# jgrss/cultionet

Hardware: AMD Instinct MI355X
Metric: train_chips_per_sec (higher is better)
Workload: dtype f32

## Files before the change

### cultionet_amd/csrc/cn_norm.hip

```cpp
#include "cn_common.h"

#define BN_SPLIT_MAX 256
#define BN_SPLIT_GROUP 64

__global__ __launch_bounds__(256) void cn_bn_partial_kernel(const float* __restrict__ x, long xbs, int B, int C,
                                                           int L, int splits, double* __restrict__ part, int vec4) {
  __shared__ double scratch[4];
  const int c = blockIdx.x, sp = blockIdx.y;
  double s = 0.0, ss = 0.0;
  if (vec4) {
    const int L4 = L >> 2;
    const int per = (L4 + splits - 1) / splits;
    const int beg = sp * per;
    const int end = (beg + per < L4) ? beg + per : L4;
    for (int b = 0; b < B; ++b) {
      const float4* xp = reinterpret_cast<const float4*>(x + b * xbs + (long)c * L);
      for (int l = beg + threadIdx.x; l < end; l += 256) {
        const float4 v = xp[l];
        s += ((double)v.x + (double)v.y) + ((double)v.z + (double)v.w);
        ss += (double)v.x * v.x + (double)v.y * v.y + (double)v.z * v.z + (double)v.w * v.w;
      }
    }
  } else {
    const int per = (L + splits - 1) / splits;
// ... 21 lines not shown
  __shared__ double scratch[4];
  double a = 0.0, b = 0.0;
  for (int i = threadIdx.x; i < splits; i += 256) {
    a += part[((long)c * splits + i) * 2 + 0];
    b += part[((long)c * splits + i) * 2 + 1];
  }
  s = cn_block_sum<double, 256>(a, scratch);
  ss = cn_block_sum<double, 256>(b, scratch);
}

__global__ void cn_bn_eval_stats_kernel(const float* __restrict__ running_mean, const float* __restrict__ running_var,
                                        int C, float eps, float* __restrict__ mean, float* __restrict__ rstd) {
  const int c = blockIdx.x * blockDim.x + threadIdx.x;
  if (c >= C) return;
  mean[c] = running_mean[c];
  rstd[c] = 1.0f / sqrtf(running_var[c] + eps);
}

__global__ __launch_bounds__(256) void cn_bn_apply_kernel(const float* __restrict__ x, long xbs,
                                                         float* __restrict__ mean, float* __restrict__ rstd,
                                                         const float* __restrict__ gamma,
                                                         const float* __restrict__ beta,
                                                         const float* __restrict__ res, long rbs,
                                                         float* __restrict__ y, long ybs, int B, int C, int L, int act,
                                                         const double* __restrict__ part, int splits, double count,
                                                         float eps, float momentum, float* __restrict__ running_mean,
                                                         float* __restrict__ running_var) {
  const int c = blockIdx.y, b = blockIdx.z;
  float m, rs;
  if (part != nullptr) {
    double s, ss;
    cn_bn_sum_parts(part, c, splits, s, ss);
    const double md = s / count;
    double var = ss / count - md * md;
    if (var < 0.0) var = 0.0;
    m = (float)md;
    rs = (float)(1.0 / sqrt(var + (double)eps));
    if (blockIdx.x == 0 && b == 0 && threadIdx.x == 0) {
      mean[c] = m;
      rstd[c] = rs;
      if (running_mean != nullptr) {
        const double unbiased = count > 1.0 ? var * count / (count - 1.0) : var;
        running_mean[c] = (1.f - momentum) * running_mean[c] + momentum * m;
        running_var[c] = (1.f - momentum) * running_var[c] + momentum * (float)unbiased;
      }
    }
  } else {
    m = mean[c];
    rs = rstd[c];
  }
  const float sc = gamma[c] * rs, be = beta[c];
  const long r0 = (long)c * L;
  const float* xp = x + b * xbs + r0;
  const float* rp = res ? res + b * rbs + r0 : nullptr;
  float* yp = y + b * ybs + r0;
  for (int l = blockIdx.x * 256 + threadIdx.x; l < L; l += gridDim.x * 256) {
    float z = (xp[l] - m) * sc + be;
    if (act == 1) z = cn_silu(z);
    if (rp) z += rp[l];
    yp[l] = z;
  }
}

__global__ __launch_bounds__(256) void cn_bn_bwd_partial_kernel(const float* __restrict__ x, long xbs,
                                                               const float* __restrict__ dy, long dybs,
                                                               const float* __restrict__ mean,
                                                               const float* __restrict__ rstd,
                                                               const float* __restrict__ gamma,
                                                               const float* __restrict__ beta, int B, int C, int L,
                                                               int act, int splits, double* __restrict__ part,
                                                               int vec4) {
  __shared__ double scratch[4];
  const int c = blockIdx.x, sp = blockIdx.y;
  const float m = mean[c], rs = rstd[c], ga = gamma[c], be = beta[c];
  double s1 = 0.0, s2 = 0.0;
  auto term = [&](float xv, float dv) {
    const float xh = (xv - m) * rs;
    float dz = dv;
    if (act == 1) dz *= cn_silu_grad(ga * xh + be);
    s1 += dz;
    s2 += (double)dz * xh;
  };
  if (vec4) {
    const int L4 = L >> 2;
    const int per = (L4 + splits - 1) / splits;
    const int beg = sp * per;
    const int end = (beg + per < L4) ? beg + per : L4;
    for (int b = 0; b < B; ++b) {
      const float4* xp = reinterpret_cast<const float4*>(x + b * xbs + (long)c * L);
      const float4* dp = reinterpret_cast<const float4*>(dy + b * dybs + (long)c * L);
      for (int l = beg + threadIdx.x; l < end; l += 256) {
        const float4 xv = xp[l], dv = dp[l];
        term(xv.x, dv.x); term(xv.y, dv.y); term(xv.z, dv.z); term(xv.w, dv.w);
      }
    }
  } else {
    const int per = (L + splits - 1) / splits;
    const int beg = sp * per;
    const int end = (beg + per < L) ? beg + per : L;
    for (int b = 0; b < B; ++b) {
      const float* xp = x + b * xbs + (long)c * L;
      const float* dp = dy + b * dybs + (long)c * L;
      for (int l = beg + threadIdx.x; l < end; l += 256) term(xp[l], dp[l]);
    }
  }
  s1 = cn_block_sum<double, 256>(s1, scratch);
  s2 = cn_block_sum<double, 256>(s2, scratch);
  if (threadIdx.x == 0) {
    part[((long)c * splits + sp) * 2 + 0] = s1;
    part[((long)c * splits + sp) * 2 + 1] = s2;
  }
}

__global__ __launch_bounds__(256) void cn_bn_bwd_apply_kernel(const float* __restrict__ x, long xbs,
                                                             const float* __restrict__ dy, long dybs,
                                                             const float* __restrict__ mean,
                                                             const float* __restrict__ rstd,
                                                             const float* __restrict__ gamma,
                                                             const float* __restrict__ beta,
                                                             const double* __restrict__ part, int splits,
                                                             double count, int training,
                                                             float* __restrict__ dgamma, float* __restrict__ dbeta,
                                                             int accumulate_params, float* __restrict__ dx, long dxbs,
                                                             int B, int C, int L, int act, int accumulate) {
  const int c = blockIdx.y, b = blockIdx.z;
  double s1, s2;
  cn_bn_sum_parts(part, c, splits, s1, s2);
  if (blockIdx.x == 0 && b == 0 && threadIdx.x == 0) {
    if (accumulate_params) {
      dgamma[c] += (float)s2;
      dbeta[c] += (float)s1;
    } else {
      dgamma[c] = (float)s2;
      dbeta[c] = (float)s1;
    }
  }
  if (dx == nullptr) return;
  const float m = mean[c], rs = rstd[c], ga = gamma[c], be = beta[c];
  const float c1 = training ? (float)(s1 / count) : 0.f, c2 = training ? (float)(s2 / count) : 0.f;
  const long r0 = (long)c * L;
  const float* xp = x + b * xbs + r0;
  const float* dp = dy + b * dybs + r0;
  float* dxp = dx + b * dxbs + r0;
  for (int l = blockIdx.x * 256 + threadIdx.x; l < L; l += gridDim.x * 256) {
    const float xh = (xp[l] - m) * rs;
    float dz = dp[l];
    if (act == 1) dz *= cn_silu_grad(ga * xh + be);
    float g = (dz - c1 - xh * c2) * (ga * rs);
    if (accumulate) g += dxp[l];
    dxp[l] = g;
  }
}

template <int NV>
__global__ __launch_bounds__(256) void cn_bn_fused_fwd_kernel(const float* __restrict__ x, long xbs,
                                                             float* __restrict__ mean, float* __restrict__ rstd,
                                                             const float* __restrict__ gamma,
                                                             const float* __restrict__ beta,
                                                             const float* __restrict__ res, long rbs,
                                                             float* __restrict__ y, long ybs, int B, int C, int L,
                                                             int act, float eps, float momentum,
                                                             float* __restrict__ running_mean,
                                                             float* __restrict__ running_var) {
  __shared__ double scratch[4];
  const int c = blockIdx.x, n = B * L;
  float v[NV];
  double s = 0.0, ss = 0.0;
#pragma unroll
  for (int k = 0; k < NV; ++k) {
    const int i = threadIdx.x + k * 256;
    v[k] = 0.f;
    if (i < n) {
      const int b = i / L, l = i - b * L;
      v[k] = x[b * xbs + (long)c * L + l];
      s += v[k];
      ss += (double)v[k] * v[k];
    }
  }
  s = cn_block_sum<double, 256>(s, scratch);
  ss = cn_block_sum<double, 256>(ss, scratch);
  const double count = (double)n;
  const double md = s / count;
  double var = ss / count - md * md;
  if (var < 0.0) var = 0.0;
  const float m = (float)md, rs = (float)(1.0 / sqrt(var + (double)eps));
  if (threadIdx.x == 0) {
    mean[c] = m;
    rstd[c] = rs;
    if (running_mean != nullptr) {
      const double unbiased = count > 1.0 ? var * count / (count - 1.0) : var;
      running_mean[c] = (1.f - momentum) * running_mean[c] + momentum * m;
      running_var[c] = (1.f - momentum) * running_var[c] + momentum * (float)unbiased;
    }
  }
  const float sc = gamma[c] * rs, be = beta[c];
#pragma unroll
  for (int k = 0; k < NV; ++k) {
    const int i = threadIdx.x + k * 256;
    if (i < n) {
      const int b = i / L, l = i - b * L;
      float z = (v[k] - m) * sc + be;
      if (act == 1) z = cn_silu(z);
      if (res) z += res[b * rbs + (long)c * L + l];
      y[b * ybs + (long)c * L + l] = z;
    }
  }
}

template <int NV>
__global__ __launch_bounds__(256) void cn_bn_fused_bwd_kernel(const float* __restrict__ x, long xbs,
                                                             const float* __restrict__ dy, long dybs,
                                                             const float* __restrict__ mean,
                                                             const float* __restrict__ rstd,
                                                             const float* __restrict__ gamma,
                                                             const float* __restrict__ beta, int training,
                                                             float* __restrict__ dgamma, float* __restrict__ dbeta,
                                                             int accumulate_params, float* __restrict__ dx, long dxbs,
                                                             int B, int C, int L, int act, int accumulate) {
  __shared__ double scratch[4];
  const int c = blockIdx.x, n = B * L;
  const float m = mean[c], rs = rstd[c], ga = gamma[c], be = beta[c];
  float xh[NV], dz[NV];
  double s1 = 0.0, s2 = 0.0;
#pragma unroll
  for (int k = 0; k < NV; ++k) {
    const int i = threadIdx.x + k * 256;
    xh[k] = 0.f;
    dz[k] = 0.f;
    if (i < n) {
      const int b = i / L, l = i - b * L;
      xh[k] = (x[b * xbs + (long)c * L + l] - m) * rs;
      float d = dy[b * dybs + (long)c * L + l];
      if (act == 1) d *= cn_silu_grad(ga * xh[k] + be);
      dz[k] = d;
      s1 += d;
      s2 += (double)d * xh[k];
    }
  }
  s1 = cn_block_sum<double, 256>(s1, scratch);
  s2 = cn_block_sum<double, 256>(s2, scratch);
  if (threadIdx.x == 0) {
    if (accumulate_params) {
      dgamma[c] += (float)s2;
      dbeta[c] += (float)s1;
    } else {
      dgamma[c] = (float)s2;
      dbeta[c] = (float)s1;
    }
  }
  if (dx == nullptr) return;
  const double count = (double)n;
  const float c1 = training ? (float)(s1 / count) : 0.f, c2 = training ? (float)(s2 / count) : 0.f;
#pragma unroll
  for (int k = 0; k < NV; ++k) {
    const int i = threadIdx.x + k * 256;
    if (i < n) {
      const int b = i / L, l = i - b * L;
      float g = (dz[k] - c1 - xh[k] * c2) * (ga * rs);
      float* o = dx + b * dxbs + (long)c * L + l;
      if (accumulate) g += *o;
      *o = g;
    }
  }
}

#define BN_FUSED_MAX (8 * 256)

static int bn_splits_wide(int C, long L) {
  int s = (2048 + C - 1) / C;
  const long maxs = (L + 511) / 512;
  if (s > maxs) s = (int)maxs;
  if (s > BN_SPLIT_MAX) s = BN_SPLIT_MAX;
  if (s < 1) s = 1;
  return s;
}

static int bn_splits(int C, long L) {
  int s = (1024 + C - 1) / C;
  const long maxs = (L + 511) / 512;
  if (s > maxs) s = (int)maxs;
  if (s > BN_SPLIT_GROUP) s = BN_SPLIT_GROUP;
  if (s < 1) s = 1;
  return s;
}

static dim3 plane_grid(int B, int C, int L) {
  int bx = (L + 1023) / 1024;
  if (bx < 1) bx = 1;
  return dim3(bx, C, B);
}

extern "C" int cn_bn_workspace_doubles(int C) { return C * BN_SPLIT_MAX * 2; }

extern "C" int cn_bn_act_fwd_f32(const float* x, long xbs, const float* gamma, const float* beta,
                                 float* running_mean, float* running_var, const float* res, long rbs, float* y,
                                 long ybs, float* mean, float* rstd, double* ws, int B, int C, int L, int training,
                                 float momentum, float eps, int act, void* stream_) {
  hipStream_t stream = (hipStream_t)stream_;
  if (B <= 0 || C <= 0 || L <= 0) return CN_OK;
  if (training && (long)B * L <= BN_FUSED_MAX && C >= 32) {
#define CN_BN_FWD(NV_)                                                                                               \
  CN_LAUNCH((cn_bn_fused_fwd_kernel<NV_>), dim3(C), dim3(256), 0, stream, x, xbs, mean, rstd, gamma, beta, res, \
                     rbs, y, ybs, B, C, L, act, eps, momentum, running_mean, running_var)
    CN_BN_FWD(8);
#undef CN_BN_FWD
    return cn_check_launch();
  }
  if (training) {
    const int splits = bn_splits_wide(C, L);
    CN_LAUNCH(cn_bn_partial_kernel, dim3(C, splits), dim3(256), 0, stream, x, xbs, B, C, L, splits, ws,
                       (int)(L % 4 == 0 && xbs % 4 == 0 && (reinterpret_cast<uintptr_t>(x) & 15) == 0));
    CN_LAUNCH(cn_bn_apply_kernel, plane_grid(B, C, L), dim3(256), 0, stream, x, xbs, mean, rstd, gamma, beta,
                       res, rbs, y, ybs, B, C, L, act, (const double*)ws, splits, (double)B * L, eps, momentum,
                       running_mean, running_var);
  } else {
    CN_LAUNCH(cn_bn_eval_stats_kernel, dim3((C + 63) / 64), dim3(64), 0, stream, running_mean,
                       running_var, C, eps, mean, rstd);
    CN_LAUNCH(cn_bn_apply_kernel, plane_grid(B, C, L), dim3(256), 0, stream, x, xbs, mean, rstd, gamma, beta,
                       res, rbs, y, ybs, B, C, L, act, (const double*)nullptr, 0, 1.0, eps, momentum,
                       (float*)nullptr, (float*)nullptr);
  }
  return cn_check_launch();
}

extern "C" int cn_bn_act_bwd_f32(const float* x, long xbs, const float* dy, long dybs, const float* mean,
                                 const float* rstd, const float* gamma, const float* beta, float* dx, long dxbs,
                                 float* dgamma, float* dbeta, float* coef, double* ws, int B, int C, int L,
                                 int training, int act, int accumulate_dx, int accumulate_params, void* stream_) {
  hipStream_t stream = (hipStream_t)stream_;
  if (B <= 0 || C <= 0 || L <= 0) return CN_OK;
  if ((long)B * L <= BN_FUSED_MAX && C >= 32) {
#define CN_BN_BWD(NV_)                                                                                              \
  CN_LAUNCH((cn_bn_fused_bwd_kernel<NV_>), dim3(C), dim3(256), 0, stream, x, xbs, dy, dybs, mean, rstd, gamma, \
                     beta, training, dgamma, dbeta, accumulate_params, dx, dxbs, B, C, L, act, accumulate_dx)
    CN_BN_BWD(8);
#undef CN_BN_BWD
    return cn_check_launch();
  }
  const int splits = bn_splits_wide(C, L);
  CN_LAUNCH(cn_bn_bwd_partial_kernel, dim3(C, splits), dim3(256), 0, stream, x, xbs, dy, dybs, mean, rstd,
                     gamma, beta, B, C, L, act, splits, ws,
                     (int)(L % 4 == 0 && xbs % 4 == 0 && dybs % 4 == 0 &&
                           ((reinterpret_cast<uintptr_t>(x) | reinterpret_cast<uintptr_t>(dy)) & 15) == 0));
  (void)coef;
  CN_LAUNCH(cn_bn_bwd_apply_kernel, dx != nullptr ? plane_grid(B, C, L) : dim3(1, C, 1), dim3(256), 0,
                     stream, x, xbs, dy, dybs, mean, rstd, gamma, beta, (const double*)ws, splits, (double)B * L,
                     training, dgamma, dbeta, accumulate_params, dx, dxbs, B, C, L, act, accumulate_dx);
  return cn_check_launch();
}

#define BN_MAX_GROUPS 4
struct CnBnGroupArgs {
  const float* x[BN_MAX_GROUPS];
  const float* gamma[BN_MAX_GROUPS];
  const float* beta[BN_MAX_GROUPS];
  float* mean[BN_MAX_GROUPS];
  float* rstd[BN_MAX_GROUPS];
  float* running_mean[BN_MAX_GROUPS];
  float* running_var[BN_MAX_GROUPS];
  float* y[BN_MAX_GROUPS];
  const float* dy[BN_MAX_GROUPS];
  float* dx[BN_MAX_GROUPS];
  float* dgamma[BN_MAX_GROUPS];
  float* dbeta[BN_MAX_GROUPS];
  int accumulate_dx[BN_MAX_GROUPS];
  long xbs, ybs, dybs, dxbs, rbs;
  const float* res;
  int G, B, C, L, act, splits, training, sum_outputs, accumulate_params;
  int vec4;
  float eps, momentum;
  double* part;
};

__global__ __launch_bounds__(256) void cn_bn_group_partial_kernel(const CnBnGroupArgs a) {
  __shared__ double scratch[4];
  const int c = blockIdx.x, sp = blockIdx.y, g = blockIdx.z;
  double s = 0.0, ss = 0.0;
  if (a.vec4) {
    const int L4 = a.L >> 2;
    const int per = (L4 + a.splits - 1) / a.splits;
    const int beg = sp * per;
    const int end = (beg + per < L4) ? beg + per : L4;
    for (int b = 0; b < a.B; ++b) {
      const float4* xp = reinterpret_cast<const float4*>(a.x[g] + b * a.xbs + (long)c * a.L);
      for (int l = beg + threadIdx.x; l < end; l += 256) {
        const float4 v = xp[l];
        s += ((double)v.x + (double)v.y) + ((double)v.z + (double)v.w);
        ss += (double)v.x * v.x + (double)v.y * v.y + (double)v.z * v.z + (double)v.w * v.w;
      }
    }
  } else {
    const int per = (a.L + a.splits - 1) / a.splits;
    const int beg = sp * per;
    const int end = (beg + per < a.L) ? beg + per : a.L;
    for (int b = 0; b < a.B; ++b) {
      const float* xp = a.x[g] + b * a.xbs + (long)c * a.L;
      for (int l = beg + threadIdx.x; l < end; l += 256) {
        const float v = xp[l];
        s += v;
        ss += (double)v * v;
      }
    }
  }
  s = cn_block_sum<double, 256>(s, scratch);
  ss = cn_block_sum<double, 256>(ss, scratch);
  if (threadIdx.x == 0) {
    double* p = a.part + (((long)g * a.C + c) * a.splits + sp) * 2;
    p[0] = s;
    p[1] = ss;
  }
}

__global__ __launch_bounds__(256) void cn_bn_group_apply_kernel(const CnBnGroupArgs a) {
  const int c = blockIdx.y, b = blockIdx.z;
  float m[BN_MAX_GROUPS], sc[BN_MAX_GROUPS], be[BN_MAX_GROUPS];
  const double count = (double)a.B * a.L;
#pragma unroll
  for (int g = 0; g < BN_MAX_GROUPS; ++g) {
    m[g] = sc[g] = be[g] = 0.f;
    if (g < a.G) {
      float rs;
      if (a.training) {
        double s = 0.0, ss = 0.0;
        const double* p = a.part + ((long)g * a.C + c) * a.splits * 2;
        for (int i = 0; i < a.splits; ++i) {
          s += p[2 * i];
          ss += p[2 * i + 1];
        }
        const double md = s / count;
        double var = ss / count - md * md;
        if (var < 0.0) var = 0.0;
        m[g] = (float)md;
        rs = (float)(1.0 / sqrt(var + (double)a.eps));
        if (blockIdx.x == 0 && b == 0 && threadIdx.x == 0) {
          a.mean[g][c] = m[g];
          a.rstd[g][c] = rs;
          if (a.running_mean[g] != nullptr) {
            const double unbiased = count > 1.0 ? var * count / (count - 1.0) : var;
            a.running_mean[g][c] = (1.f - a.momentum) * a.running_mean[g][c] + a.momentum * m[g];
            a.running_var[g][c] = (1.f - a.momentum) * a.running_var[g][c] + a.momentum * (float)unbiased;
          }
        }
      } else {
        m[g] = a.running_mean[g][c];
        rs = 1.0f / sqrtf(a.running_var[g][c] + a.eps);
        if (blockIdx.x == 0 && b == 0 && threadIdx.x == 0) {
          a.mean[g][c] = m[g];
          a.rstd[g][c] = rs;
        }
      }
      sc[g] = a.gamma[g][c] * rs;
      be[g] = a.beta[g][c];
    }
  }
  const long r0 = (long)c * a.L;
  const float* rp = a.res ? a.res + b * a.rbs + r0 : nullptr;
  if (a.vec4) {
    const float4 z4 = {0.f, 0.f, 0.f, 0.f};
    for (int l = blockIdx.x * 256 + threadIdx.x; l < (a.L >> 2); l += gridDim.x * 256) {
      float4 acc = rp ? reinterpret_cast<const float4*>(rp)[l] : z4;
#pragma unroll
      for (int g = 0; g < BN_MAX_GROUPS; ++g) {
        if (g < a.G) {
          const float4 xv = reinterpret_cast<const float4*>(a.x[g] + b * a.xbs + r0)[l];
          float4 z;
          z.x = (xv.x - m[g]) * sc[g] + be[g];
          z.y = (xv.y - m[g]) * sc[g] + be[g];
          z.z = (xv.z - m[g]) * sc[g] + be[g];
          z.w = (xv.w - m[g]) * sc[g] + be[g];
          if (a.act == 1) { z.x = cn_silu(z.x); z.y = cn_silu(z.y); z.z = cn_silu(z.z); z.w = cn_silu(z.w); }
          if (a.sum_outputs) { acc.x += z.x; acc.y += z.y; acc.z += z.z; acc.w += z.w; }
          else reinterpret_cast<float4*>(a.y[g] + b * a.ybs + r0)[l] = z;
        }
      }
      if (a.sum_outputs) reinterpret_cast<float4*>(a.y[0] + b * a.ybs + r0)[l] = acc;
    }
    return;
  }
  for (int l = blockIdx.x * 256 + threadIdx.x; l < a.L; l += gridDim.x * 256) {
    float acc = rp ? rp[l] : 0.f;
#pragma unroll
    for (int g = 0; g < BN_MAX_GROUPS; ++g) {
      if (g < a.G) {
        float z = (a.x[g][b * a.xbs + r0 + l] - m[g]) * sc[g] + be[g];
        if (a.act == 1) z = cn_silu(z);
        if (a.sum_outputs) acc += z;
        else a.y[g][b * a.ybs + r0 + l] = z;
      }
    }
    if (a.sum_outputs) a.y[0][b * a.ybs + r0 + l] = acc;
  }
}

__global__ __launch_bounds__(256) void cn_bn_group_bwd_partial_kernel(const CnBnGroupArgs a) {
  __shared__ double scratch[4];
  const int c = blockIdx.x, sp = blockIdx.y, g = blockIdx.z;
  const float m = a.mean[g][c], rs = a.rstd[g][c], ga = a.gamma[g][c], be = a.beta[g][c];
  double s1 = 0.0, s2 = 0.0;
  auto term = [&](float xv, float dv) {
    const float xh = (xv - m) * rs;
    float dz = dv;
    if (a.act == 1) dz *= cn_silu_grad(ga * xh + be);
    s1 += dz;
    s2 += (double)dz * xh;
  };
  if (a.vec4) {
    const int L4 = a.L >> 2;
    const int per = (L4 + a.splits - 1) / a.splits;
    const int beg = sp * per;
    const int end = (beg + per < L4) ? beg + per : L4;
    for (int b = 0; b < a.B; ++b) {
      const float4* xp = reinterpret_cast<const float4*>(a.x[g] + b * a.xbs + (long)c * a.L);
      const float4* dp = reinterpret_cast<const float4*>(a.dy[g] + b * a.dybs + (long)c * a.L);
      for (int l = beg + threadIdx.x; l < end; l += 256) {
        const float4 xv = xp[l], dv = dp[l];
        term(xv.x, dv.x); term(xv.y, dv.y); term(xv.z, dv.z); term(xv.w, dv.w);
      }
    }
  } else {
    const int per = (a.L + a.splits - 1) / a.splits;
    const int beg = sp * per;
    const int end = (beg + per < a.L) ? beg + per : a.L;
    for (int b = 0; b < a.B; ++b) {
      const float* xp = a.x[g] + b * a.xbs + (long)c * a.L;
      const float* dp = a.dy[g] + b * a.dybs + (long)c * a.L;
      for (int l = beg + threadIdx.x; l < end; l += 256) term(xp[l], dp[l]);
    }
  }
  s1 = cn_block_sum<double, 256>(s1, scratch);
  s2 = cn_block_sum<double, 256>(s2, scratch);
  if (threadIdx.x == 0) {
    double* p = a.part + (((long)g * a.C + c) * a.splits + sp) * 2;
    p[0] = s1;
    p[1] = s2;
  }
}

__global__ __launch_bounds__(256) void cn_bn_group_bwd_apply_kernel(const CnBnGroupArgs a, int bx_per_group) {
  const int g = blockIdx.x / bx_per_group, bx = blockIdx.x - g * bx_per_group;
  const int c = blockIdx.y, b = blockIdx.z;
  double s1 = 0.0, s2 = 0.0;
  const double* p = a.part + ((long)g * a.C + c) * a.splits * 2;
  for (int i = 0; i < a.splits; ++i) {
    s1 += p[2 * i];
    s2 += p[2 * i + 1];
  }
  if (bx == 0 && b == 0 && threadIdx.x == 0) {
    if (a.accumulate_params) {
      a.dgamma[g][c] += (float)s2;
      a.dbeta[g][c] += (float)s1;
    } else {
      a.dgamma[g][c] = (float)s2;
      a.dbeta[g][c] = (float)s1;
    }
  }
  if (a.dx[g] == nullptr) return;
  const double count = (double)a.B * a.L;
  const float m = a.mean[g][c], rs = a.rstd[g][c], ga = a.gamma[g][c], be = a.beta[g][c];
  const float c1 = a.training ? (float)(s1 / count) : 0.f, c2 = a.training ? (float)(s2 / count) : 0.f;
  const long r0 = (long)c * a.L;
  const float* xp = a.x[g] + b * a.xbs + r0;
  const float* dp = a.dy[g] + b * a.dybs + r0;
  float* dxp = a.dx[g] + b * a.dxbs + r0;
  const int acc = a.accumulate_dx[g];
  const float gs = ga * rs;
  auto grad = [&](float xv, float dv, float prev) {
    const float xh = (xv - m) * rs;
    float dz = dv;
    if (a.act == 1) dz *= cn_silu_grad(ga * xh + be);
    float gr = (dz - c1 - xh * c2) * gs;
    if (acc) gr += prev;
    return gr;
  };
  if (a.vec4) {
    const float4* x4 = reinterpret_cast<const float4*>(xp);
    const float4* d4 = reinterpret_cast<const float4*>(dp);
    float4* o4 = reinterpret_cast<float4*>(dxp);
    const float4 z = {0.f, 0.f, 0.f, 0.f};
    for (int l = bx * 256 + threadIdx.x; l < (a.L >> 2); l += bx_per_group * 256) {
      const float4 xv = x4[l], dv = d4[l];
      const float4 pv = acc ? o4[l] : z;
      float4 o;
      o.x = grad(xv.x, dv.x, pv.x); o.y = grad(xv.y, dv.y, pv.y);
      o.z = grad(xv.z, dv.z, pv.z); o.w = grad(xv.w, dv.w, pv.w);
      o4[l] = o;
    }
    return;
  }
  for (int l = bx * 256 + threadIdx.x; l < a.L; l += bx_per_group * 256) dxp[l] = grad(xp[l], dp[l], acc ? dxp[l] : 0.f);
}

extern "C" int cn_bn_act_group_fwd_f32(int G, const float* const* xs, long xbs, const float* const* gammas,
                                       const float* const* betas, float* const* running_means,
                                       float* const* running_vars, const float* res, long rbs, float* const* ys,
                                       long ybs, float* const* means, float* const* rstds, double* ws, int B, int C,
                                       int L, int training, float momentum, float eps, int act, int sum_outputs,
                                       void* stream_) {
  hipStream_t stream = (hipStream_t)stream_;
  if (G < 1 || G > BN_MAX_GROUPS || (!sum_outputs && res != nullptr)) return CN_ERR_ARG;
  if (B <= 0 || C <= 0 || L <= 0) return CN_OK;
  CnBnGroupArgs a = {};
  for (int g = 0; g < G; ++g) {
    a.x[g] = xs[g]; a.gamma[g] = gammas[g]; a.beta[g] = betas[g];
    a.running_mean[g] = running_means ? running_means[g] : nullptr;
    a.running_var[g] = running_vars ? running_vars[g] : nullptr;
    if (!training && (a.running_mean[g] == nullptr || a.running_var[g] == nullptr)) return CN_ERR_ARG;
    a.mean[g] = means[g]; a.rstd[g] = rstds[g];
    a.y[g] = sum_outputs ? ys[0] : ys[g];
  }
  a.xbs = xbs; a.ybs = ybs; a.rbs = rbs; a.res = res;
  a.G = G; a.B = B; a.C = C; a.L = L; a.act = act; a.training = training; a.sum_outputs = sum_outputs;
  a.eps = eps; a.momentum = momentum; a.part = ws;
  a.splits = bn_splits(C * G, L);
  a.vec4 = (L % 4 == 0) && xbs % 4 == 0 && ybs % 4 == 0 && (res == nullptr || rbs % 4 == 0) &&
           (reinterpret_cast<uintptr_t>(res) & 15) == 0;
  for (int g = 0; g < G; ++g)
    if ((reinterpret_cast<uintptr_t>(a.x[g]) | reinterpret_cast<uintptr_t>(a.y[g])) & 15) a.vec4 = 0;
  if (training)
    CN_LAUNCH(cn_bn_group_partial_kernel, dim3(C, a.splits, G), dim3(256), 0, stream, a);
  CN_LAUNCH(cn_bn_group_apply_kernel, plane_grid(B, C, L), dim3(256), 0, stream, a);
  return cn_check_launch();
}

extern "C" int cn_bn_act_group_bwd_f32(int G, const float* const* xs, long xbs, const float* const* dys, long dybs,
                                       const float* const* means, const float* const* rstds,
                                       const float* const* gammas, const float* const* betas, float* const* dxs,
                                       long dxbs, const int* accumulate_dx, float* const* dgammas,
                                       float* const* dbetas, double* ws, int B, int C, int L, int training, int act,
                                       int accumulate_params, void* stream_) {
  hipStream_t stream = (hipStream_t)stream_;
  if (G < 1 || G > BN_MAX_GROUPS) return CN_ERR_ARG;
  if (B <= 0 || C <= 0 || L <= 0) return CN_OK;
  CnBnGroupArgs a = {};
  for (int g = 0; g < G; ++g) {
    a.x[g] = xs[g]; a.dy[g] = dys[g]; a.gamma[g] = gammas[g]; a.beta[g] = betas[g];
    a.mean[g] = const_cast<float*>(means[g]); a.rstd[g] = const_cast<float*>(rstds[g]);
    a.dx[g] = dxs ? dxs[g] : nullptr; a.dgamma[g] = dgammas[g]; a.dbeta[g] = dbetas[g];
    a.accumulate_dx[g] = accumulate_dx ? accumulate_dx[g] : 0;
  }
  a.xbs = xbs; a.dybs = dybs; a.dxbs = dxbs;
  a.G = G; a.B = B; a.C = C; a.L = L; a.act = act; a.training = training; a.accumulate_params = accumulate_params;
  a.part = ws;
  a.splits = bn_splits(C * G, L);
  a.vec4 = (L % 4 == 0) && xbs % 4 == 0 && dybs % 4 == 0 && dxbs % 4 == 0;
  for (int g = 0; g < G; ++g)
    if ((reinterpret_cast<uintptr_t>(a.x[g]) | reinterpret_cast<uintptr_t>(a.dy[g]) |
         reinterpret_cast<uintptr_t>(a.dx[g])) & 15)
      a.vec4 = 0;
  CN_LAUNCH(cn_bn_group_bwd_partial_kernel, dim3(C, a.splits, G), dim3(256), 0, stream, a);
  const dim3 pg = plane_grid(B, C, L);
  CN_LAUNCH(cn_bn_group_bwd_apply_kernel, dim3(pg.x * G, pg.y, pg.z), dim3(256), 0, stream, a, (int)pg.x);
  return cn_check_launch();
}

__global__ __launch_bounds__(256) void cn_channel_sum_kernel(const float* __restrict__ x, long xbs, int B, int C,
                                                            int L, int splits, float* __restrict__ out) {
  __shared__ double scratch[4];
  const int c = blockIdx.x, sp = blockIdx.y;
  const int per = (L + splits - 1) / splits;
  const int beg = sp * per;
  const int end = (beg + per < L) ? beg + per : L;
  double s = 0.0;
  for (int b = 0; b < B; ++b) {
    const float* xp = x + b * xbs + (long)c * L;
    for (int l = beg + threadIdx.x; l < end; l += 256) s += xp[l];
  }
  s = cn_block_sum<double, 256>(s, scratch);
  if (threadIdx.x == 0) atomicAdd(out + c, (float)s);
}

extern "C" int cn_channel_sum_f32(const float* x, long xbs, int B, int C, int L, float* out, int accumulate,
                                  void* stream_) {
  hipStream_t stream = (hipStream_t)stream_;
  if (C <= 0) return CN_OK;
  if (!accumulate && hipMemsetAsync(out, 0, sizeof(float) * C, stream) != hipSuccess) return CN_ERR_LAUNCH;
  const int splits = bn_splits(C, L);
  CN_LAUNCH(cn_channel_sum_kernel, dim3(C, splits), dim3(256), 0, stream, x, xbs, B, C, L, splits, out);
  return cn_check_launch();
}

__global__ __launch_bounds__(256) void cn_ln_fwd_kernel(const float* __restrict__ x, long xbs,
                                                       const float* __restrict__ w, const float* __restrict__ bvec,
                                                       const float* __restrict__ res, long rbs,
                                                       float* __restrict__ y, long ybs, float* __restrict__ mu,
                                                       float* __restrict__ rstd, int B, int C, int L, float eps) {
  const long p = blockIdx.x * 256L + threadIdx.x;
  if (p >= (long)B * L) return;
  const long b = p / L, l = p - b * L;
  const float* xp = x + b * xbs + l;
  float s = 0.f;
  for (int c = 0; c < C; ++c) s += xp[(long)c * L];
  const float m = s / C;
  float v = 0.f;
  for (int c = 0; c < C; ++c) {
    const float d = xp[(long)c * L] - m;
    v += d * d;
  }
  const float rs = 1.0f / sqrtf(v / C + eps);
  mu[p] = m;
  rstd[p] = rs;
  float* yp = y + b * ybs + l;
  const float* rp = res ? res + b * rbs + l : nullptr;
  for (int c = 0; c < C; ++c) {
    float o = (xp[(long)c * L] - m) * rs * w[c] + bvec[c];
    if (rp) o += rp[(long)c * L];
    yp[(long)c * L] = o;
  }
}

template <int MAXC>
__global__ __launch_bounds__(256) void cn_ln_bwd_kernel(const float* __restrict__ x, long xbs,
                                                       const float* __restrict__ dy, long dybs,
                                                       const float* __restrict__ w, const float* __restrict__ mu,
                                                       const float* __restrict__ rstd, float* __restrict__ dx,
                                                       long dxbs, float* __restrict__ dw, float* __restrict__ db,
                                                       int B, int C, int L, int accumulate_dx) {
  __shared__ float red[2][4][MAXC];
  const long p = blockIdx.x * 256L + threadIdx.x;
  const bool ok = p < (long)B * L;
  const int lane = threadIdx.x & 63, wid = threadIdx.x >> 6;
  long b = 0, l = 0;
  float m = 0.f, rs = 0.f;
  if (ok) {
    b = p / L;
    l = p - b * L;
    m = mu[p];
    rs = rstd[p];
  }
  const float* xp = x + b * xbs + l;
  const float* dp = dy + b * dybs + l;
  float s1 = 0.f, s2 = 0.f;
  for (int c = 0; c < C; ++c) {
    float g = 0.f, xh = 0.f, d = 0.f;
    if (ok) {
      d = dp[(long)c * L];
      xh = (xp[(long)c * L] - m) * rs;
      g = d * w[c];
    }
    s1 += g;
    s2 += g * xh;
    const float dwv = cn_wave_sum(d * xh);
    const float dbv = cn_wave_sum(d);
    if (lane == 0) {
      red[0][wid][c] = dwv;
      red[1][wid][c] = dbv;
    }
  }
  if (ok) {
    const float a1 = s1 / C, a2 = s2 / C;
    float* dxp = dx + b * dxbs + l;
    for (int c = 0; c < C; ++c) {
      const float xh = (xp[(long)c * L] - m) * rs;
      float g = rs * (dp[(long)c * L] * w[c] - a1 - xh * a2);
      if (accumulate_dx) g += dxp[(long)c * L];
      dxp[(long)c * L] = g;
    }
  }
  __syncthreads();
  for (int c = threadIdx.x; c < C; c += 256) {
    atomicAdd(dw + c, red[0][0][c] + red[0][1][c] + red[0][2][c] + red[0][3][c]);
    atomicAdd(db + c, red[1][0][c] + red[1][1][c] + red[1][2][c] + red[1][3][c]);
  }
}

template <int CPW>
__global__ __launch_bounds__(256) void cn_ln_fwd_reg_kernel(const float* __restrict__ x, long xbs,
                                                           const float* __restrict__ w,
                                                           const float* __restrict__ bvec,
                                                           const float* __restrict__ res, long rbs,
                                                           float* __restrict__ y, long ybs, float* __restrict__ mu,
                                                           float* __restrict__ rstd, int B, int C, int L, float eps) {
  __shared__ float red[2][4][64];
  const int lane = threadIdx.x & 63, wid = threadIdx.x >> 6;
  const long p = blockIdx.x * 64L + lane;
  const bool ok = p < (long)B * L;
  const long b = ok ? p / L : 0, l = ok ? p - b * L : 0;
  const int c0 = wid * CPW;
  const float* xp = x + b * xbs + l + (long)c0 * L;
  const float* rp = res ? res + b * rbs + l + (long)c0 * L : nullptr;
  float xv[CPW], rv[CPW];
  float s = 0.f;
#pragma unroll
  for (int i = 0; i < CPW; ++i) {
    xv[i] = (ok && c0 + i < C) ? xp[(long)i * L] : 0.f;
    s += xv[i];
  }
#pragma unroll
  for (int i = 0; i < CPW; ++i) rv[i] = (rp && ok && c0 + i < C) ? rp[(long)i * L] : 0.f;
  red[0][wid][lane] = s;
  __syncthreads();
  const float m = (red[0][0][lane] + red[0][1][lane] + red[0][2][lane] + red[0][3][lane]) / C;
  float v = 0.f;
#pragma unroll
  for (int i = 0; i < CPW; ++i) {
    const float d = xv[i] - m;
    v += (c0 + i < C) ? d * d : 0.f;
  }
  red[1][wid][lane] = v;
  __syncthreads();
  const float rs = 1.0f / sqrtf((red[1][0][lane] + red[1][1][lane] + red[1][2][lane] + red[1][3][lane]) / C + eps);
  if (!ok) return;
  if (wid == 0) {
    mu[p] = m;
// ... 194 lines not shown
```

Baseline: 391.3.

## Add register-resident single-pass batchnorm kernels for single and grouped paths

Replaces the small fused BN kernels (limited to B*L <= 2048) with generalized register-resident forward and backward kernels. They hold a whole channel in registers across 512-1024 threads with optional float4 vectorization and compute the statistics and the apply step in one launch. This extends to the grouped BN paths, including summed multi-group outputs. The aim is to remove the two-kernel partial+apply sequence and its second read of x for mid-sized planes, in exchange for heavy register pressure, lower occupancy and reduced parallelism when there are few channels.

```diff
diff --git a/cultionet_amd/csrc/cn_norm.hip b/cultionet_amd/csrc/cn_norm.hip
--- a/cultionet_amd/csrc/cn_norm.hip
+++ b/cultionet_amd/csrc/cn_norm.hip
@@ -197,120 +197,6 @@
   }
 }
 
-template <int NV>
-__global__ __launch_bounds__(256) void cn_bn_fused_fwd_kernel(const float* __restrict__ x, long xbs,
-                                                             float* __restrict__ mean, float* __restrict__ rstd,
-                                                             const float* __restrict__ gamma,
-                                                             const float* __restrict__ beta,
-                                                             const float* __restrict__ res, long rbs,
-                                                             float* __restrict__ y, long ybs, int B, int C, int L,
-                                                             int act, float eps, float momentum,
-                                                             float* __restrict__ running_mean,
-                                                             float* __restrict__ running_var) {
-  __shared__ double scratch[4];
-  const int c = blockIdx.x, n = B * L;
-  float v[NV];
-  double s = 0.0, ss = 0.0;
-#pragma unroll
-  for (int k = 0; k < NV; ++k) {
-    const int i = threadIdx.x + k * 256;
-    v[k] = 0.f;
-    if (i < n) {
-      const int b = i / L, l = i - b * L;
-      v[k] = x[b * xbs + (long)c * L + l];
-      s += v[k];
-      ss += (double)v[k] * v[k];
-    }
-  }
-  s = cn_block_sum<double, 256>(s, scratch);
-  ss = cn_block_sum<double, 256>(ss, scratch);
-  const double count = (double)n;
-  const double md = s / count;
-  double var = ss / count - md * md;
-  if (var < 0.0) var = 0.0;
-  const float m = (float)md, rs = (float)(1.0 / sqrt(var + (double)eps));
-  if (threadIdx.x == 0) {
-    mean[c] = m;
-    rstd[c] = rs;
-    if (running_mean != nullptr) {
-      const double unbiased = count > 1.0 ? var * count / (count - 1.0) : var;
-      running_mean[c] = (1.f - momentum) * running_mean[c] + momentum * m;
-      running_var[c] = (1.f - momentum) * running_var[c] + momentum * (float)unbiased;
-    }
-  }
-  const float sc = gamma[c] * rs, be = beta[c];
-#pragma unroll
-  for (int k = 0; k < NV; ++k) {
-    const int i = threadIdx.x + k * 256;
-    if (i < n) {
-      const int b = i / L, l = i - b * L;
-      float z = (v[k] - m) * sc + be;
-      if (act == 1) z = cn_silu(z);
-      if (res) z += res[b * rbs + (long)c * L + l];
-      y[b * ybs + (long)c * L + l] = z;
-    }
-  }
-}
-
-template <int NV>
-__global__ __launch_bounds__(256) void cn_bn_fused_bwd_kernel(const float* __restrict__ x, long xbs,
-                                                             const float* __restrict__ dy, long dybs,
-                                                             const float* __restrict__ mean,
-                                                             const float* __restrict__ rstd,
-                                                             const float* __restrict__ gamma,
-                                                             const float* __restrict__ beta, int training,
-                                                             float* __restrict__ dgamma, float* __restrict__ dbeta,
-                                                             int accumulate_params, float* __restrict__ dx, long dxbs,
-                                                             int B, int C, int L, int act, int accumulate) {
-  __shared__ double scratch[4];
-  const int c = blockIdx.x, n = B * L;
-  const float m = mean[c], rs = rstd[c], ga = gamma[c], be = beta[c];
-  float xh[NV], dz[NV];
-  double s1 = 0.0, s2 = 0.0;
-#pragma unroll
-  for (int k = 0; k < NV; ++k) {
-    const int i = threadIdx.x + k * 256;
-    xh[k] = 0.f;
-    dz[k] = 0.f;
-    if (i < n) {
-      const int b = i / L, l = i - b * L;
-      xh[k] = (x[b * xbs + (long)c * L + l] - m) * rs;
-      float d = dy[b * dybs + (long)c * L + l];
-      if (act == 1) d *= cn_silu_grad(ga * xh[k] + be);
-      dz[k] = d;
-      s1 += d;
-      s2 += (double)d * xh[k];
-    }
-  }
-  s1 = cn_block_sum<double, 256>(s1, scratch);
-  s2 = cn_block_sum<double, 256>(s2, scratch);
-  if (threadIdx.x == 0) {
-    if (accumulate_params) {
-      dgamma[c] += (float)s2;
-      dbeta[c] += (float)s1;
-    } else {
-      dgamma[c] = (float)s2;
-      dbeta[c] = (float)s1;
-    }
-  }
-  if (dx == nullptr) return;
-  const double count = (double)n;
-  const float c1 = training ? (float)(s1 / count) : 0.f, c2 = training ? (float)(s2 / count) : 0.f;
-#pragma unroll
-  for (int k = 0; k < NV; ++k) {
-    const int i = threadIdx.x + k * 256;
-    if (i < n) {
-      const int b = i / L, l = i - b * L;
-      float g = (dz[k] - c1 - xh[k] * c2) * (ga * rs);
-      float* o = dx + b * dxbs + (long)c * L + l;
-      if (accumulate) g += *o;
-      *o = g;
-    }
-  }
-}
-
-#define BN_FUSED_MAX (8 * 256)
-
 static int bn_splits_wide(int C, long L) {
   int s = (2048 + C - 1) / C;
   const long maxs = (L + 511) / 512;
@@ -336,63 +222,6 @@
 }
 
 extern "C" int cn_bn_workspace_doubles(int C) { return C * BN_SPLIT_MAX * 2; }
-
-extern "C" int cn_bn_act_fwd_f32(const float* x, long xbs, const float* gamma, const float* beta,
-                                 float* running_mean, float* running_var, const float* res, long rbs, float* y,
-                                 long ybs, float* mean, float* rstd, double* ws, int B, int C, int L, int training,
-                                 float momentum, float eps, int act, void* stream_) {
-  hipStream_t stream = (hipStream_t)stream_;
-  if (B <= 0 || C <= 0 || L <= 0) return CN_OK;
-  if (training && (long)B * L <= BN_FUSED_MAX && C >= 32) {
-#define CN_BN_FWD(NV_)                                                                                               \
-  CN_LAUNCH((cn_bn_fused_fwd_kernel<NV_>), dim3(C), dim3(256), 0, stream, x, xbs, mean, rstd, gamma, beta, res, \
-                     rbs, y, ybs, B, C, L, act, eps, momentum, running_mean, running_var)
-    CN_BN_FWD(8);
-#undef CN_BN_FWD
-    return cn_check_launch();
-  }
-  if (training) {
-    const int splits = bn_splits_wide(C, L);
-    CN_LAUNCH(cn_bn_partial_kernel, dim3(C, splits), dim3(256), 0, stream, x, xbs, B, C, L, splits, ws,
-                       (int)(L % 4 == 0 && xbs % 4 == 0 && (reinterpret_cast<uintptr_t>(x) & 15) == 0));
-    CN_LAUNCH(cn_bn_apply_kernel, plane_grid(B, C, L), dim3(256), 0, stream, x, xbs, mean, rstd, gamma, beta,
-                       res, rbs, y, ybs, B, C, L, act, (const double*)ws, splits, (double)B * L, eps, momentum,
-                       running_mean, running_var);
-  } else {
-    CN_LAUNCH(cn_bn_eval_stats_kernel, dim3((C + 63) / 64), dim3(64), 0, stream, running_mean,
-                       running_var, C, eps, mean, rstd);
-    CN_LAUNCH(cn_bn_apply_kernel, plane_grid(B, C, L), dim3(256), 0, stream, x, xbs, mean, rstd, gamma, beta,
-                       res, rbs, y, ybs, B, C, L, act, (const double*)nullptr, 0, 1.0, eps, momentum,
-                       (float*)nullptr, (float*)nullptr);
-  }
-  return cn_check_launch();
-}
-
-extern "C" int cn_bn_act_bwd_f32(const float* x, long xbs, const float* dy, long dybs, const float* mean,
-                                 const float* rstd, const float* gamma, const float* beta, float* dx, long dxbs,
-                                 float* dgamma, float* dbeta, float* coef, double* ws, int B, int C, int L,
-                                 int training, int act, int accumulate_dx, int accumulate_params, void* stream_) {
-  hipStream_t stream = (hipStream_t)stream_;
-  if (B <= 0 || C <= 0 || L <= 0) return CN_OK;
-  if ((long)B * L <= BN_FUSED_MAX && C >= 32) {
-#define CN_BN_BWD(NV_)                                                                                              \
-  CN_LAUNCH((cn_bn_fused_bwd_kernel<NV_>), dim3(C), dim3(256), 0, stream, x, xbs, dy, dybs, mean, rstd, gamma, \
-                     beta, training, dgamma, dbeta, accumulate_params, dx, dxbs, B, C, L, act, accumulate_dx)
-    CN_BN_BWD(8);
-#undef CN_BN_BWD
-    return cn_check_launch();
-  }
-  const int splits = bn_splits_wide(C, L);
-  CN_LAUNCH(cn_bn_bwd_partial_kernel, dim3(C, splits), dim3(256), 0, stream, x, xbs, dy, dybs, mean, rstd,
-                     gamma, beta, B, C, L, act, splits, ws,
-                     (int)(L % 4 == 0 && xbs % 4 == 0 && dybs % 4 == 0 &&
-                           ((reinterpret_cast<uintptr_t>(x) | reinterpret_cast<uintptr_t>(dy)) & 15) == 0));
-  (void)coef;
-  CN_LAUNCH(cn_bn_bwd_apply_kernel, dx != nullptr ? plane_grid(B, C, L) : dim3(1, C, 1), dim3(256), 0,
-                     stream, x, xbs, dy, dybs, mean, rstd, gamma, beta, (const double*)ws, splits, (double)B * L,
-                     training, dgamma, dbeta, accumulate_params, dx, dxbs, B, C, L, act, accumulate_dx);
-  return cn_check_launch();
-}
 
 #define BN_MAX_GROUPS 4
 struct CnBnGroupArgs {
@@ -416,6 +245,358 @@
   float eps, momentum;
   double* part;
 };
+
+#define BN_RES_CHUNK 4
+template <bool V4> struct CnBnUnit { typedef float type; };
+template <> struct CnBnUnit<true> { typedef float4 type; };
+
+__device__ __forceinline__ void cn_bn_clear(float& v) { v = 0.f; }
+__device__ __forceinline__ void cn_bn_clear(float4& v) { v.x = v.y = v.z = v.w = 0.f; }
+__device__ __forceinline__ void cn_bn_stat(float v, double& s, double& ss) {
+  s += v;
+  ss += (double)v * v;
+}
+__device__ __forceinline__ void cn_bn_stat(const float4& v, double& s, double& ss) {
+  s += ((double)v.x + (double)v.y) + ((double)v.z + (double)v.w);
+  ss += (double)v.x * v.x + (double)v.y * v.y + (double)v.z * v.z + (double)v.w * v.w;
+}
+template <class F> __device__ __forceinline__ float cn_bn_map(float a, float b, F f) { return f(a, b); }
+template <class F> __device__ __forceinline__ float4 cn_bn_map(const float4& a, const float4& b, F f) {
+  float4 r;
+  r.x = f(a.x, b.x); r.y = f(a.y, b.y); r.z = f(a.z, b.z); r.w = f(a.w, b.w);
+  return r;
+}
+
+template <int NT>
+__device__ __forceinline__ void cn_bn_block_sum2(double& a, double& b, double* scratch) {
+  asm volatile("" : "+v"(a), "+v"(b));
+  a = cn_wave_sum(a);
+  b = cn_wave_sum(b);
+  const int lane = threadIdx.x & 63, wid = threadIdx.x >> 6;
+  __syncthreads();
+  if (lane == 0) {
+    scratch[2 * wid] = a;
+    scratch[2 * wid + 1] = b;
+  }
+  __syncthreads();
+  a = b = 0.0;
+#pragma unroll
+  for (int i = 0; i < NT / 64; ++i) {
+    a += scratch[2 * i];
+    b += scratch[2 * i + 1];
+  }
+}
+
+struct CnBnWalk {
+  int b, l, n, qt, rt;
+  __device__ __forceinline__ CnBnWalk(int t, int T, int n_) : n(n_) {
+    asm volatile("" : "+v"(t));
+    b = t / n_;
+    l = t - b * n_;
+    qt = T / n_;
+    rt = T - qt * n_;
+  }
+  __device__ __forceinline__ void next() {
+    b += qt;
+    l += rt;
+    if (l >= n) {
+      l -= n;
+      ++b;
+    }
+  }
+};
+
+template <int T, int NV, int GS, bool V4>
+__global__ __launch_bounds__(T) void cn_bn_res_fwd_kernel(const CnBnGroupArgs a) {
+  typedef typename CnBnUnit<V4>::type V;
+  constexpr int U = V4 ? 4 : 1;
+  __shared__ double scratch[2 * (T / 64)];
+  const int c = blockIdx.x, g0 = GS == 1 ? blockIdx.y : 0;
+  const int n = a.L / U;
+  const long r0 = (long)c * a.L;
+  V v[GS][NV];
+  {
+    CnBnWalk w(threadIdx.x, T, n);
+#pragma unroll
+    for (int k = 0; k < NV; ++k) {
+      if (w.b < a.B) {
+        const long o = w.b * a.xbs + r0 + w.l * U;
+#pragma unroll
+        for (int g = 0; g < GS; ++g) v[g][k] = *reinterpret_cast<const V*>(a.x[g0 + g] + o);
+      } else {
+#pragma unroll
+        for (int g = 0; g < GS; ++g) cn_bn_clear(v[g][k]);
+      }
+      w.next();
+    }
+  }
+  const double count = (double)a.B * a.L;
+  float m[GS], sc[GS], be[GS];
+#pragma unroll
+  for (int g = 0; g < GS; ++g) {
+    double s = 0.0, ss = 0.0;
+#pragma unroll
+    for (int k = 0; k < NV; ++k) cn_bn_stat(v[g][k], s, ss);
+    cn_bn_block_sum2<T>(s, ss, scratch);
+    const double md = s / count;
+    double var = ss / count - md * md;
+    if (var < 0.0) var = 0.0;
+    m[g] = (float)md;
+    const float rs = (float)(1.0 / sqrt(var + (double)a.eps));
+    if (threadIdx.x == 0) {
+      a.mean[g0 + g][c] = m[g];
+      a.rstd[g0 + g][c] = rs;
+      if (a.running_mean[g0 + g] != nullptr) {
+        const double unbiased = count > 1.0 ? var * count / (count - 1.0) : var;
+        float* rm = a.running_mean[g0 + g];
+        float* rv = a.running_var[g0 + g];
+        rm[c] = (1.f - a.momentum) * rm[c] + a.momentum * m[g];
+        rv[c] = (1.f - a.momentum) * rv[c] + a.momentum * (float)unbiased;
+      }
+    }
+    sc[g] = a.gamma[g0 + g][c] * rs;
+    be[g] = a.beta[g0 + g][c];
+  }
+  const bool has_res = a.res != nullptr;
+  const int act = a.act;
+  float* yp = a.y[g0];
+  CnBnWalk w(threadIdx.x, T, n);
+#pragma unroll
+  for (int k0 = 0; k0 < NV; k0 += BN_RES_CHUNK) {
+    V rr[BN_RES_CHUNK];
+    if (has_res) {
+      CnBnWalk wr = w;
+#pragma unroll
+      for (int j = 0; j < BN_RES_CHUNK; ++j) {
+        if (k0 + j < NV && wr.b < a.B) rr[j] = *reinterpret_cast<const V*>(a.res + wr.b * a.rbs + r0 + wr.l * U);
+        wr.next();
+      }
+    }
+#pragma unroll
+    for (int j = 0; j < BN_RES_CHUNK; ++j) {
+      const int k = k0 + j;
+      if (k < NV) {
+        if (w.b < a.B) {
+          V acc;
+#pragma unroll
+          for (int g = 0; g < GS; ++g) {
+            const float mg = m[g], sg = sc[g], bg = be[g];
+            const V z = cn_bn_map(v[g][k], v[g][k], [&](float xv, float) {
+              const float t = (xv - mg) * sg + bg;
+              return act == 1 ? cn_silu(t) : t;
+            });
+            if (g == 0) {
+              if (has_res) acc = cn_bn_map(rr[j], z, [](float r, float f) { return r + f; });
+              else if (a.sum_outputs) acc = cn_bn_map(z, z, [](float f, float) { return 0.f + f; });
+              else acc = z;
+            } else {
+              acc = cn_bn_map(acc, z, [](float p, float f) { return p + f; });
+            }
+          }
+          *reinterpret_cast<V*>(yp + w.b * a.ybs + r0 + w.l * U) = acc;
+        }
+        w.next();
+      }
+    }
+  }
+}
+
+template <int T, int NV, bool V4>
+__global__ __launch_bounds__(T) void cn_bn_res_bwd_kernel(const CnBnGroupArgs a) {
+  typedef typename CnBnUnit<V4>::type V;
+  constexpr int U = V4 ? 4 : 1;
+  __shared__ double scratch[2 * (T / 64)];
+  const int c = blockIdx.x, g = blockIdx.y;
+  const int n = a.L / U;
+  const long r0 = (long)c * a.L;
+  V xh[NV], dz[NV];
+  {
+    CnBnWalk w(threadIdx.x, T, n);
+    const float* xp = a.x[g];
+    const float* dyp = a.dy[g];
+#pragma unroll
+    for (int k = 0; k < NV; ++k) {
+      if (w.b < a.B) {
+        xh[k] = *reinterpret_cast<const V*>(xp + w.b * a.xbs + r0 + w.l * U);
+        dz[k] = *reinterpret_cast<const V*>(dyp + w.b * a.dybs + r0 + w.l * U);
+      } else {
+        cn_bn_clear(xh[k]);
+        cn_bn_clear(dz[k]);
+      }
+      w.next();
+    }
+  }
+  const double count = (double)a.B * a.L;
+  const int act = a.act;
+  const float m = a.mean[g][c], rs = a.rstd[g][c], ga = a.gamma[g][c], be = a.beta[g][c];
+  double s1 = 0.0, s2 = 0.0;
+#pragma unroll
+  for (int k = 0; k < NV; ++k) {
+    xh[k] = cn_bn_map(xh[k], xh[k], [&](float xv, float) { return (xv - m) * rs; });
+    dz[k] = cn_bn_map(dz[k], xh[k], [&](float dv, float h) {
+      if (act == 1) dv *= cn_silu_grad(ga * h + be);
+      s1 += dv;
+      s2 += (double)dv * h;
+      return dv;
+    });
+  }
+  cn_bn_block_sum2<T>(s1, s2, scratch);
+  if (threadIdx.x == 0) {
+    if (a.accumulate_params) {
+      a.dgamma[g][c] += (float)s2;
+      a.dbeta[g][c] += (float)s1;
+    } else {
+      a.dgamma[g][c] = (float)s2;
+      a.dbeta[g][c] = (float)s1;
+    }
+  }
+  float* dxp = a.dx[g];
+  if (dxp == nullptr) return;
+  const bool acc = a.accumulate_dx[g] != 0;
+  const float k1 = a.training ? (float)(s1 / count) : 0.f, k2 = a.training ? (float)(s2 / count) : 0.f, kg = ga * rs;
+  CnBnWalk w(threadIdx.x, T, n);
+#pragma unroll
+  for (int k0 = 0; k0 < NV; k0 += BN_RES_CHUNK) {
+    V pv[BN_RES_CHUNK];
+    if (acc) {
+      CnBnWalk wr = w;
+#pragma unroll
+      for (int j = 0; j < BN_RES_CHUNK; ++j) {
+        if (k0 + j < NV && wr.b < a.B) pv[j] = *reinterpret_cast<const V*>(dxp + wr.b * a.dxbs + r0 + wr.l * U);
+        wr.next();
+      }
+    }
+#pragma unroll
+    for (int j = 0; j < BN_RES_CHUNK; ++j) {
+      const int k = k0 + j;
+      if (k < NV) {
+        if (w.b < a.B) {
+          V o = cn_bn_map(dz[k], xh[k], [&](float d, float h) { return (d - k1 - h * k2) * kg; });
+          if (acc) o = cn_bn_map(o, pv[j], [](float gr, float prev) { return gr + prev; });
+          *reinterpret_cast<V*>(dxp + w.b * a.dxbs + r0 + w.l * U) = o;
+        }
+        w.next();
+      }
+    }
+  }
+}
+
+struct CnBnPlan {
+  int T, NV, GS;
+};
+static const struct { int T, NV, gs_fwd, bwd; } BN_RES_SHAPES[] = {{512, 4, 3, 1}, {1024, 5, 3, 1}, {1024, 10, 2, 1},
+                                                                    {1024, 20, 1, 0}};
+#define BN_RES_FULL_BLOCKS 128
+#define BN_RES_SMALL 20480
+
+static CnBnPlan bn_resident_plan(bool backward, int G, bool summed, int B, int C, int L, bool v4) {
+  const CnBnPlan none = {0, 0, 0};
+  const long units = (long)B * (L / (v4 ? 4 : 1));
+  const int GS = (!backward && summed) ? G : 1;
+  for (const auto& s : BN_RES_SHAPES) {
+    if ((backward ? !s.bwd : GS > s.gs_fwd) || (long)s.T * s.NV < units) continue;
+#ifndef CN_BN_RESIDENT_ALL
+    if ((long)C * (GS == 1 ? G : 1) < BN_RES_FULL_BLOCKS && (long)B * L * GS > BN_RES_SMALL) break;
+#endif
+    const CnBnPlan p = {s.T, s.NV, GS};
+    return p;
+  }
+  return none;
+}
+
+template <bool BWD, int T, int NV, int GS>
+static void bn_resident_launch_one(const CnBnGroupArgs& a, hipStream_t stream) {
+  const dim3 grid(a.C, GS == 1 ? a.G : 1);
+  if constexpr (BWD) {
+    if (a.vec4) CN_LAUNCH((cn_bn_res_bwd_kernel<T, NV, true>), grid, dim3(T), 0, stream, a);
+    else CN_LAUNCH((cn_bn_res_bwd_kernel<T, NV, false>), grid, dim3(T), 0, stream, a);
+  } else {
+    if (a.vec4) CN_LAUNCH((cn_bn_res_fwd_kernel<T, NV, GS, true>), grid, dim3(T), 0, stream, a);
+    else CN_LAUNCH((cn_bn_res_fwd_kernel<T, NV, GS, false>), grid, dim3(T), 0, stream, a);
+  }
+}
+
+template <bool BWD>
+static bool bn_resident_launch(const CnBnPlan& p, const CnBnGroupArgs& a, hipStream_t stream) {
+#define CN_BN_RES(T_, NV_, GS_)                           \
+  if (p.T == T_ && p.NV == NV_ && p.GS == GS_) {          \
+    bn_resident_launch_one<BWD, T_, NV_, GS_>(a, stream); \
+    return true;                                          \
+  }
+  CN_BN_RES(512, 4, 1) CN_BN_RES(1024, 5, 1) CN_BN_RES(1024, 10, 1)
+  if constexpr (!BWD) {
+    CN_BN_RES(512, 4, 2) CN_BN_RES(512, 4, 3) CN_BN_RES(1024, 5, 2) CN_BN_RES(1024, 5, 3) CN_BN_RES(1024, 10, 2)
+    CN_BN_RES(1024, 20, 1)
+  }
+#undef CN_BN_RES
+  return false;
+}
+
+extern "C" int cn_bn_act_fwd_f32(const float* x, long xbs, const float* gamma, const float* beta,
+                                 float* running_mean, float* running_var, const float* res, long rbs, float* y,
+                                 long ybs, float* mean, float* rstd, double* ws, int B, int C, int L, int training,
+                                 float momentum, float eps, int act, void* stream_) {
+  hipStream_t stream = (hipStream_t)stream_;
+  if (B <= 0 || C <= 0 || L <= 0) return CN_OK;
+  if (training) {
+    CnBnGroupArgs a = {};
+    a.x[0] = x; a.gamma[0] = gamma; a.beta[0] = beta; a.mean[0] = mean; a.rstd[0] = rstd;
+    a.running_mean[0] = running_mean; a.running_var[0] = running_mean != nullptr ? running_var : nullptr;
+    a.y[0] = y; a.res = res;
+    a.xbs = xbs; a.ybs = ybs; a.rbs = rbs;
+    a.G = 1; a.B = B; a.C = C; a.L = L; a.act = act; a.training = 1; a.sum_outputs = res != nullptr;
+    a.eps = eps; a.momentum = momentum;
+    a.vec4 = L % 4 == 0 && xbs % 4 == 0 && ybs % 4 == 0 && (res == nullptr || rbs % 4 == 0) &&
+             ((reinterpret_cast<uintptr_t>(x) | reinterpret_cast<uintptr_t>(y) | reinterpret_cast<uintptr_t>(res)) & 15) == 0;
+    const CnBnPlan p = bn_resident_plan(false, 1, false, B, C, L, a.vec4 != 0);
+    if (p.NV != 0 && bn_resident_launch<false>(p, a, stream)) return cn_check_launch();
+  }
+  if (training) {
+    const int splits = bn_splits_wide(C, L);
+    CN_LAUNCH(cn_bn_partial_kernel, dim3(C, splits), dim3(256), 0, stream, x, xbs, B, C, L, splits, ws,
+                       (int)(L % 4 == 0 && xbs % 4 == 0 && (reinterpret_cast<uintptr_t>(x) & 15) == 0));
+    CN_LAUNCH(cn_bn_apply_kernel, plane_grid(B, C, L), dim3(256), 0, stream, x, xbs, mean, rstd, gamma, beta,
+                       res, rbs, y, ybs, B, C, L, act, (const double*)ws, splits, (double)B * L, eps, momentum,
+                       running_mean, running_var);
+  } else {
+    CN_LAUNCH(cn_bn_eval_stats_kernel, dim3((C + 63) / 64), dim3(64), 0, stream, running_mean,
+                       running_var, C, eps, mean, rstd);
+    CN_LAUNCH(cn_bn_apply_kernel, plane_grid(B, C, L), dim3(256), 0, stream, x, xbs, mean, rstd, gamma, beta,
+                       res, rbs, y, ybs, B, C, L, act, (const double*)nullptr, 0, 1.0, eps, momentum,
+                       (float*)nullptr, (float*)nullptr);
+  }
+  return cn_check_launch();
+}
+
+extern "C" int cn_bn_act_bwd_f32(const float* x, long xbs, const float* dy, long dybs, const float* mean,
+                                 const float* rstd, const float* gamma, const float* beta, float* dx, long dxbs,
+                                 float* dgamma, float* dbeta, float* coef, double* ws, int B, int C, int L,
+                                 int training, int act, int accumulate_dx, int accumulate_params, void* stream_) {
+  hipStream_t stream = (hipStream_t)stream_;
+  if (B <= 0 || C <= 0 || L <= 0) return CN_OK;
+  {
+    CnBnGroupArgs a = {};
+    a.x[0] = x; a.dy[0] = dy; a.gamma[0] = gamma; a.beta[0] = beta;
+    a.mean[0] = const_cast<float*>(mean); a.rstd[0] = const_cast<float*>(rstd);
+    a.dx[0] = dx; a.dgamma[0] = dgamma; a.dbeta[0] = dbeta; a.accumulate_dx[0] = accumulate_dx;
+    a.xbs = xbs; a.dybs = dybs; a.dxbs = dxbs;
+    a.G = 1; a.B = B; a.C = C; a.L = L; a.act = act; a.training = training; a.accumulate_params = accumulate_params;
+    a.vec4 = L % 4 == 0 && xbs % 4 == 0 && dybs % 4 == 0 && (dx == nullptr || dxbs % 4 == 0) &&
+             ((reinterpret_cast<uintptr_t>(x) | reinterpret_cast<uintptr_t>(dy) | reinterpret_cast<uintptr_t>(dx)) & 15) == 0;
+    const CnBnPlan p = bn_resident_plan(true, 1, false, B, C, L, a.vec4 != 0);
+    if (p.NV != 0 && bn_resident_launch<true>(p, a, stream)) return cn_check_launch();
+  }
+  const int splits = bn_splits_wide(C, L);
+  CN_LAUNCH(cn_bn_bwd_partial_kernel, dim3(C, splits), dim3(256), 0, stream, x, xbs, dy, dybs, mean, rstd,
+                     gamma, beta, B, C, L, act, splits, ws,
+                     (int)(L % 4 == 0 && xbs % 4 == 0 && dybs % 4 == 0 &&
+                           ((reinterpret_cast<uintptr_t>(x) | reinterpret_cast<uintptr_t>(dy)) & 15) == 0));
+  (void)coef;
+  CN_LAUNCH(cn_bn_bwd_apply_kernel, dx != nullptr ? plane_grid(B, C, L) : dim3(1, C, 1), dim3(256), 0,
+                     stream, x, xbs, dy, dybs, mean, rstd, gamma, beta, (const double*)ws, splits, (double)B * L,
+                     training, dgamma, dbeta, accumulate_params, dx, dxbs, B, C, L, act, accumulate_dx);
+  return cn_check_launch();
+}
 
 __global__ __launch_bounds__(256) void cn_bn_group_partial_kernel(const CnBnGroupArgs a) {
   __shared__ double scratch[4];
@@ -661,6 +842,10 @@
            (reinterpret_cast<uintptr_t>(res) & 15) == 0;
   for (int g = 0; g < G; ++g)
     if ((reinterpret_cast<uintptr_t>(a.x[g]) | reinterpret_cast<uintptr_t>(a.y[g])) & 15) a.vec4 = 0;
+  if (training) {
+    const CnBnPlan p = bn_resident_plan(false, G, sum_outputs != 0, B, C, L, a.vec4 != 0);
+    if (p.NV != 0 && bn_resident_launch<false>(p, a, stream)) return cn_check_launch();
+  }
   if (training)
     CN_LAUNCH(cn_bn_group_partial_kernel, dim3(C, a.splits, G), dim3(256), 0, stream, a);
   CN_LAUNCH(cn_bn_group_apply_kernel, plane_grid(B, C, L), dim3(256), 0, stream, a);
@@ -692,8 +877,10 @@
     if ((reinterpret_cast<uintptr_t>(a.x[g]) | reinterpret_cast<uintptr_t>(a.dy[g]) |
          reinterpret_cast<uintptr_t>(a.dx[g])) & 15)
       a.vec4 = 0;
+  const CnBnPlan p = bn_resident_plan(true, G, false, B, C, L, a.vec4 != 0);
+  if (p.NV != 0 && bn_resident_launch<true>(p, a, stream)) return cn_check_launch();
+  const dim3 pg = plane_grid(B, C, L);
   CN_LAUNCH(cn_bn_group_bwd_partial_kernel, dim3(C, a.splits, G), dim3(256), 0, stream, a);
-  const dim3 pg = plane_grid(B, C, L);
   CN_LAUNCH(cn_bn_group_bwd_apply_kernel, dim3(pg.x * G, pg.y, pg.z), dim3(256), 0, stream, a, (int)pg.x);
   return cn_check_launch();
 }
```

Result: faster. 402.0, median of 6 (+2.7%).
